# Hippogriff/parsenet-codebase

Hardware: AMD Instinct MI355X
Metric: shapes/sec fwd+bwd on 10k-pt clouds (higher is better)
Workload: dtype f32; 1 GPU; cfg5: ParSeNet e2e (seg + mean-shift 10 it. + per-segment spline/primitive fit + Chamfer/residual), 10k pts, batch 4 per GPU, fwd+bwd+allreduce+Adam; batch_per_gpu=4, points=10000, k=80, parallelism=dp1, global_batch=4

## Files before the change

include/parsenet_hip.h:

```cpp
#ifndef PARSENET_HIP_H
#define PARSENET_HIP_H

#include <stddef.h>
#include <stdint.h>

#ifdef __cplusplus
extern "C" {
#endif

#define PN_OK 0
#define PN_ERR_ARG (-1)
#define PN_ERR_HIP (-2)
#define PN_ERR_WORKSPACE (-3)
#define PN_ERR_UNSUPPORTED (-4)

const char* pn_last_error(void);
int pn_abi_version(void);

void pn_prof_enable(int on);
void pn_prof_reset(void);
int pn_prof_count(void);
int pn_prof_get(int i, char* name, int name_len, double* total_ms, long long* calls);

size_t pn_knn_workspace(int B, int C, int N, int k);
// ... 68 lines not shown
                                int64_t* nearest, void* workspace, size_t workspace_bytes, void* stream);
size_t pn_gemm_x3_weight_image_bytes(int M, int K);
size_t pn_gemm_x3_points_image_bytes(int B, int C, int N);
int pn_gemm_x3_weight_image_f32(const float* w, int M, int K, int transposed, void* img, void* stream);
int pn_gemm_x3_f32(const void* img_a, const float* x, const float* bias, int B, int M, int K, int N, float* out,
                   void* workspace, size_t workspace_bytes, void* stream);
int pn_gemm_x3_cat_f32(const void* img_a, const float* const* xs, const int* cs, int nsrc, const float* bias, int B,
                       int M, int N, float* out, void* workspace, size_t workspace_bytes, void* stream);
size_t pn_gemm_x3_wgrad_workspace(int B, int M, int K, int N);
int pn_gemm_x3_wgrad_f32(const float* gy, const float* x, int B, int M, int K, int N, float* gw, float* gb,
                         void* workspace, size_t workspace_bytes, void* stream);
size_t pn_meanshift_rows_bwd_workspace(int B, int N);
int pn_meanshift_rows_bwd_f32(const float* gy, const float* y, const float* q, const float* rsum, const float* unorm,
                              const float* x, const float* bsq, int B, int N, int D, int R, float* gq, float* gx,
                              void* workspace, size_t workspace_bytes, void* stream);
int pn_meanshift_rows_scatter_add_f32(const float* g, const int64_t* rows, int B, int N, int D, int R, float* gx,
                                      void* stream);
size_t pn_meanshift_x3_plan_bytes(int B, int N);
size_t pn_meanshift_x3_plan_core_bytes(int B, int N);
int pn_kmeans_assign_f32(const float* x, const float* cen, int B, int N, int D, int K, int* lab, void* stream);
int pn_kmeans_centres_f32(const float* x, const int* lab, const float* old, int B, int N, int D, int K,
                          float* cen, void* stream);
int pn_cell_order_i32(const int* rank, const int* home, const int* fine, int B, int N, int P, int F,
                      long long* perm, void* stream);
int pn_meanshift_x3_tileinfo_f32(const float* z, int B, int N, int D, float* cen, float* rho, float* cnt,
                                 void* stream);
int pn_meanshift_x3_plan_f32(const float* cenQ, const float* rhoQ, const float* cenX, const float* rhoX,
                             const float* cntX, const float* bsq, int B, int N, float rel_eps, void* plan,
                             void* stream);
int pn_meanshift_x3_iter_fwd_plan_f32(const float* q, const void* img_x, const float* bsq, int B, int N,
// ... 208 lines not shown
```

parsenet_codebase_amd/_lib.py:

```python
import ctypes
import os

import torch

_HERE = os.path.dirname(os.path.abspath(__file__))
LIB_PATH = os.path.join(_HERE, "libparsenet_hip.so")

c_void_p = ctypes.c_void_p
c_int = ctypes.c_int
c_float = ctypes.c_float
c_size_t = ctypes.c_size_t
c_double = ctypes.c_double

ABI_VERSION = 22

SIGNATURES = {
    "pn_last_error": (ctypes.c_char_p, []),
    "pn_abi_version": (c_int, []),
    "pn_prof_enable": (None, [c_int]),
    "pn_prof_reset": (None, []),
    "pn_prof_count": (c_int, []),
    "pn_prof_get": (c_int, [c_int, ctypes.c_char_p, c_int, ctypes.POINTER(c_double),
                            ctypes.POINTER(ctypes.c_longlong)]),
    "pn_knn_workspace": (c_size_t, [c_int, c_int, c_int, c_int]),
    "pn_knn_f32": (c_int, [c_void_p, c_int, c_int, c_int, c_int, c_void_p, c_void_p, c_size_t, c_void_p]),
    "pn_knn_pn_f32": (c_int, [c_void_p, c_int, c_int, c_int, c_void_p, c_void_p, c_size_t, c_void_p]),
    "pn_knn_graph_i32": (c_int, [c_void_p, c_int, c_int, c_int, c_int, c_int, c_void_p, c_void_p, c_size_t, c_void_p]),
    "pn_knn3_ragged": (c_int, [c_void_p, c_void_p, c_int, c_int, c_int, c_int, c_void_p, c_void_p, c_void_p]),
    "pn_transpose_f32": (c_int, [c_void_p, c_void_p, c_int, c_int, c_int, c_void_p]),
# ... 55 lines not shown
                               c_void_p]),
    "pn_standardize_select_f32": (c_int, [c_void_p, c_int, c_int, c_int, c_void_p, c_void_p]),
    "pn_standardize_scale_f32": (c_int, [c_void_p, c_void_p, c_void_p, c_int, c_int, c_float, c_void_p, c_void_p,
                                         c_void_p]),
    "pn_gather_flat_f32": (c_int, [c_void_p, c_void_p, c_void_p, c_int, c_void_p, c_void_p]),
    "pn_adam_flat_f32": (c_int, [c_void_p, c_void_p, c_void_p, c_void_p, ctypes.c_longlong, ctypes.c_float,
                                 ctypes.c_float, ctypes.c_float, ctypes.c_float, c_int, c_void_p]),
    "pn_gemm_x3_cat_f32": (c_int, [c_void_p, c_void_p, c_void_p, c_int, c_void_p, c_int, c_int, c_int, c_void_p, c_void_p,
                                   c_size_t, c_void_p]),
    "pn_gemm_x3_wgrad_workspace": (c_size_t, [c_int, c_int, c_int, c_int]),
    "pn_gemm_x3_wgrad_f32": (c_int, [c_void_p, c_void_p, c_int, c_int, c_int, c_int, c_void_p, c_void_p, c_void_p,
                                     c_size_t, c_void_p]),
    "pn_meanshift_rows_bwd_workspace": (c_size_t, [c_int, c_int]),
    "pn_meanshift_rows_bwd_f32": (c_int, [c_void_p] * 7 + [c_int, c_int, c_int, c_int, c_void_p, c_void_p, c_void_p,
                                          c_size_t, c_void_p]),
    "pn_meanshift_rows_scatter_add_f32": (c_int, [c_void_p, c_void_p, c_int, c_int, c_int, c_int, c_void_p, c_void_p]),
    "pn_meanshift_x3_plan_bytes": (c_size_t, [c_int, c_int]),
    "pn_meanshift_x3_plan_core_bytes": (c_size_t, [c_int, c_int]),
    "pn_gn_max_finish_f32": (c_int, [c_void_p] * 8 + [c_int, c_int, c_int] + [c_void_p] * 5),
    "pn_gn_max_bwd_prep_f32": (c_int, [c_void_p] * 3 + [c_int, c_int] + [c_void_p] * 3),
    "pn_cell_order_i32": (c_int, [c_void_p, c_void_p, c_void_p, c_int, c_int, c_int, c_int, c_void_p, c_void_p]),
    "pn_kmeans_assign_f32": (c_int, [c_void_p, c_void_p, c_int, c_int, c_int, c_int, c_void_p, c_void_p]),
    "pn_kmeans_centres_f32": (c_int, [c_void_p, c_void_p, c_void_p, c_int, c_int, c_int, c_int, c_void_p, c_void_p]),
    "pn_meanshift_chain_order_f32": (c_int, [c_void_p, c_int, c_int, c_void_p, c_void_p]),
    "pn_meanshift_x3_tileinfo_f32": (c_int, [c_void_p, c_int, c_int, c_int, c_void_p, c_void_p, c_void_p, c_void_p]),
    "pn_meanshift_x3_plan_f32": (c_int, [c_void_p] * 6 + [c_int, c_int, c_float, c_void_p, c_void_p]),
    "pn_meanshift_x3_iter_fwd_plan_f32": (c_int, [c_void_p] * 3 + [c_int, c_int, c_int] + [c_void_p] * 5 +
                                          [c_void_p, c_void_p]),
    "pn_meanshift_x3_iter_fwd_info_f32": (c_int, [c_void_p] * 3 + [c_int, c_int, c_int] + [c_void_p] * 5 +
                                          [c_void_p] * 5),
# ... 295 lines not shown
```

parsenet_codebase_amd/csrc/error.hip:

```cpp
#include "common.h"
#include <stdarg.h>

static thread_local char g_err[512] = "";

void pn_set_error(const char* fmt, ...) {
  va_list ap;
  va_start(ap, fmt);
  vsnprintf(g_err, sizeof(g_err), fmt, ap);
  va_end(ap);
}

extern "C" const char* pn_last_error(void) { return g_err; }

extern "C" int pn_abi_version(void) { return 22; }
```

parsenet_codebase_amd/csrc/meanshift_rows.hip:

```cpp
#include "common.h"
#include <cstdlib>

#define MR_DMAX 128
#define MR_R 64
#define MR_CB 64
#define MR_LDOF(D) ((D) + 4)
#define MR_LG 68
#define MR_LOG2E 1.4426950408889634f
#define MR_LIM2 (75.0f * MR_LOG2E)

__device__ static inline float4 mr_ld4(const float* p) { return *reinterpret_cast<const float4*>(p); }
template <int NV>
__device__ static inline void mr_ldn(const float* p, float* v) {
  if constexpr (NV == 8) {
    const float4 a = mr_ld4(p), b = mr_ld4(p + 4);
    v[0] = a.x; v[1] = a.y; v[2] = a.z; v[3] = a.w;
    v[4] = b.x; v[5] = b.y; v[6] = b.z; v[7] = b.w;
  } else if constexpr (NV == 4) {
    const float4 a = mr_ld4(p);
    v[0] = a.x; v[1] = a.y; v[2] = a.z; v[3] = a.w;
  } else {
    const float2 a = *reinterpret_cast<const float2*>(p);
    v[0] = a.x; v[1] = a.y;
  }
}

template <int MR_D, int MR_LD>
__global__ __launch_bounds__(256) void pn_ms_rows_prep_kernel(const float* __restrict__ gy, const float* __restrict__ y,
                                                              const float* __restrict__ rsum, const float* __restrict__ unorm,
                                                              const float* __restrict__ bsq, int R, float* __restrict__ gu,
                                                              float* __restrict__ scal) {
  const int b = blockIdx.y;
  const int wave = threadIdx.x >> 6, lane = threadIdx.x & 63;
  const int r = blockIdx.x * 4 + wave;
  if (r >= MR_R) return;
  float u0 = 0.f, u1 = 0.f, c = 0.f, al = 0.f, ri = 0.f;
  if (r < R) {
    const size_t base = ((size_t)b * R + r) * MR_D;
    const bool lo = MR_D >= 64 || lane < MR_D;
    float y0 = 0.f, y1 = 0.f, g0 = 0.f, g1 = 0.f;
    if (lo) y0 = y[base + lane];
    if constexpr (MR_D == 128) y1 = y[base + lane + 64];
    if (lo) g0 = gy[base + lane];
    if constexpr (MR_D == 128) g1 = gy[base + lane + 64];
    const float nn = unorm[(size_t)b * R + r], rr = rsum[(size_t)b * R + r];
    const float yg = pn_wave_sum(y0 * g0 + y1 * g1);
    u0 = (g0 - y0 * yg) / nn;
    u1 = (g1 - y1 * yg) / nn;
    c = pn_wave_sum(u0 * (y0 * nn) + u1 * (y1 * nn));
    al = 1.0f / (rr * bsq[b]);
    ri = 1.0f / rr;
  }
  float* g = gu + ((size_t)b * MR_R + r) * MR_D;
  if (lane < MR_D) g[lane] = u0;
  if constexpr (MR_D == 128) g[lane + 64] = u1;
  if (lane == 0) {
    float* sp = scal + ((size_t)b * MR_R + r) * 4;
    sp[0] = c;
    sp[1] = al;
    sp[2] = ri;
    sp[3] = 0.f;
  }
}

template <int MR_D, int MR_LD>
__global__ __launch_bounds__(256) void pn_ms_rows_bwd_kernel(
    const float* __restrict__ gu, const float* __restrict__ scal, const float* __restrict__ q,
    const float* __restrict__ x, const float* __restrict__ bsq, int N, int R, int nblk, float* __restrict__ gx,
    float* __restrict__ gq_part) {
  extern __shared__ __attribute__((aligned(16))) float lds[];
  float* Xs = lds;
  float* Qs = Xs + MR_CB * MR_LD;
  float* Us = Qs + MR_R * MR_LD;
  float* GS = Us + MR_R * MR_LD;
  float* KR = GS + MR_R * MR_LG;
  float* GT = KR + MR_R * MR_LG;
  float* sc = GT + MR_CB * MR_LG;
  float* sa = sc + MR_R;
  float* sr = sa + MR_R;
  const int b = blockIdx.y, blk = blockIdx.x, tid = threadIdx.x;
  constexpr int MR_L4 = MR_D == 128 ? 5 : MR_D == 64 ? 4 : 3;

  const int j0 = blk * MR_CB;
  const float bs = bsq[b];
  const float hl = (0.5f / bs) * MR_LOG2E;
  const float* __restrict__ xb = x + (size_t)b * N * MR_D;

  for (int it = tid; it < MR_CB * (MR_D / 4); it += 256) {
    const int r = it >> MR_L4, c4 = it & (MR_D / 4 - 1);
    float4 v = make_float4(0.f, 0.f, 0.f, 0.f);
    if (j0 + r < N) v = mr_ld4(xb + (size_t)(j0 + r) * MR_D + 4 * c4);
    *reinterpret_cast<float4*>(Xs + r * MR_LD + 4 * c4) = v;
    float4 w = make_float4(0.f, 0.f, 0.f, 0.f);
    if (r < R) w = mr_ld4(q + ((size_t)b * R + r) * MR_D + 4 * c4);
    *reinterpret_cast<float4*>(Qs + r * MR_LD + 4 * c4) = w;
  }
  for (int it = tid; it < MR_R * (MR_D / 4); it += 256) {
    const int r = it >> MR_L4, c4 = it & (MR_D / 4 - 1);
    *reinterpret_cast<float4*>(Us + r * MR_LD + 4 * c4) = mr_ld4(gu + ((size_t)b * MR_R + r) * MR_D + 4 * c4);
  }
  if (tid < MR_R) {
    const float4 sv = mr_ld4(scal + ((size_t)b * MR_R + tid) * 4);
    sc[tid] = sv.x;
    sa[tid] = sv.y;
    sr[tid] = sv.z;
  }
  __syncthreads();

  {
    const int ti = tid >> 4, tj = tid & 15;
    float s[4][4], t[4][4];
#pragma unroll
    for (int a = 0; a < 4; ++a)
#pragma unroll
      for (int e = 0; e < 4; ++e) {
        s[a][e] = 0.f;
        t[a][e] = 0.f;
      }
    for (int k = 0; k < MR_D; k += 4) {
      float4 qv[4], uv[4], xv[4];
#pragma unroll
      for (int a = 0; a < 4; ++a) {
        qv[a] = mr_ld4(Qs + (ti + 16 * a) * MR_LD + k);
        uv[a] = mr_ld4(Us + (ti + 16 * a) * MR_LD + k);
        xv[a] = mr_ld4(Xs + (tj + 16 * a) * MR_LD + k);
      }
#pragma unroll
      for (int a = 0; a < 4; ++a)
#pragma unroll
        for (int e = 0; e < 4; ++e) {
          s[a][e] = __builtin_fmaf(qv[a].x, xv[e].x, s[a][e]);
          s[a][e] = __builtin_fmaf(qv[a].y, xv[e].y, s[a][e]);
          s[a][e] = __builtin_fmaf(qv[a].z, xv[e].z, s[a][e]);
          s[a][e] = __builtin_fmaf(qv[a].w, xv[e].w, s[a][e]);
          t[a][e] = __builtin_fmaf(uv[a].x, xv[e].x, t[a][e]);
          t[a][e] = __builtin_fmaf(uv[a].y, xv[e].y, t[a][e]);
          t[a][e] = __builtin_fmaf(uv[a].z, xv[e].z, t[a][e]);
          t[a][e] = __builtin_fmaf(uv[a].w, xv[e].w, t[a][e]);
        }
    }
#pragma unroll
    for (int a = 0; a < 4; ++a) {
      const int i = ti + 16 * a;
      const float ci = sc[i], ai = sa[i], ri = sr[i];
#pragma unroll
      for (int e = 0; e < 4; ++e) {
        const int j = tj + 16 * e;
        const float dist = __builtin_fmaf(-2.0f, s[a][e], 2.0f);
        const float a2 = -dist * hl;
        const float a2c = __builtin_amdgcn_fmed3f(a2, -MR_LIM2, MR_LIM2);
        float kv = __builtin_amdgcn_exp2f(a2c);
        if (j0 + j >= N) kv = 0.f;
        const float g = a2c == a2 ? kv * ((t[a][e] - ci) * ai) : 0.f;
        GS[i * MR_LG + j] = g;
        GT[j * MR_LG + i] = g;
        KR[i * MR_LG + j] = kv * ri;
      }
    }
  }
  __syncthreads();

  constexpr int NF4 = MR_D / 4;
  constexpr int RPT = MR_CB * NF4 / 256;
  const int f4 = tid & (NF4 - 1), grp = tid >> MR_L4;
  {
    float4 acc[RPT];
#pragma unroll
    for (int e = 0; e < RPT; ++e) acc[e] = make_float4(0.f, 0.f, 0.f, 0.f);
    for (int i = 0; i < MR_R; ++i) {
      const float4 qv = mr_ld4(Qs + i * MR_LD + 4 * f4);
      const float4 uv = mr_ld4(Us + i * MR_LD + 4 * f4);
      float gv[RPT], kv[RPT];
      mr_ldn<RPT>(GS + i * MR_LG + RPT * grp, gv);
      mr_ldn<RPT>(KR + i * MR_LG + RPT * grp, kv);
#pragma unroll
      for (int e = 0; e < RPT; ++e) {
        acc[e].x = __builtin_fmaf(gv[e], qv.x, acc[e].x);
        acc[e].y = __builtin_fmaf(gv[e], qv.y, acc[e].y);
        acc[e].z = __builtin_fmaf(gv[e], qv.z, acc[e].z);
        acc[e].w = __builtin_fmaf(gv[e], qv.w, acc[e].w);
        acc[e].x = __builtin_fmaf(kv[e], uv.x, acc[e].x);
        acc[e].y = __builtin_fmaf(kv[e], uv.y, acc[e].y);
        acc[e].z = __builtin_fmaf(kv[e], uv.z, acc[e].z);
        acc[e].w = __builtin_fmaf(kv[e], uv.w, acc[e].w);
// ... 1 lines not shown
    }
#pragma unroll
    for (int e = 0; e < RPT; ++e) {
      const int j = j0 + RPT * grp + e;
      if (j < N) {
        float4* o = reinterpret_cast<float4*>(gx + ((size_t)b * N + j) * MR_D + 4 * f4);
        float4 v = *o;
        v.x += acc[e].x;
        v.y += acc[e].y;
        v.z += acc[e].z;
        v.w += acc[e].w;
        *o = v;
      }
    }
  }
  {
    float4 acc[RPT];
#pragma unroll
    for (int e = 0; e < RPT; ++e) acc[e] = make_float4(0.f, 0.f, 0.f, 0.f);
    for (int j = 0; j < MR_CB; ++j) {
      const float4 xv = mr_ld4(Xs + j * MR_LD + 4 * f4);
      float gv[RPT];
      mr_ldn<RPT>(GT + j * MR_LG + RPT * grp, gv);
#pragma unroll
      for (int e = 0; e < RPT; ++e) {
        acc[e].x = __builtin_fmaf(gv[e], xv.x, acc[e].x);
        acc[e].y = __builtin_fmaf(gv[e], xv.y, acc[e].y);
        acc[e].z = __builtin_fmaf(gv[e], xv.z, acc[e].z);
        acc[e].w = __builtin_fmaf(gv[e], xv.w, acc[e].w);
      }
    }
    float* pb = gq_part + ((size_t)b * nblk + blk) * MR_R * MR_D;
#pragma unroll
    for (int e = 0; e < RPT; ++e) *reinterpret_cast<float4*>(pb + (RPT * grp + e) * MR_D + 4 * f4) = acc[e];
  }
}

template <int MR_D, int MR_LD>
__global__ __launch_bounds__(256) void pn_ms_rows_reduce_kernel(const float* __restrict__ gq_part, int R, int nblk,
                                                                float* __restrict__ gq) {
  const int b = blockIdx.y;
  const int e = blockIdx.x * 256 + threadIdx.x;
  if (e >= R * (MR_D / 4)) return;
  const float* p = gq_part + (size_t)b * nblk * MR_R * MR_D + 4 * e;
  float4 s = make_float4(0.f, 0.f, 0.f, 0.f);
  int k = 0;
  for (; k + 8 <= nblk; k += 8) {
    float4 v[8];
#pragma unroll
    for (int u = 0; u < 8; ++u) v[u] = mr_ld4(p + (size_t)(k + u) * MR_R * MR_D);
#pragma unroll
    for (int u = 0; u < 8; ++u) {
      s.x += v[u].x;
      s.y += v[u].y;
      s.z += v[u].z;
      s.w += v[u].w;
    }
  }
  for (; k < nblk; ++k) {
    const float4 v = mr_ld4(p + (size_t)k * MR_R * MR_D);
    s.x += v.x;
    s.y += v.y;
    s.z += v.z;
    s.w += v.w;
  }
  *reinterpret_cast<float4*>(gq + (size_t)b * R * MR_D + 4 * e) = s;
}

template <int MR_D, int MR_LD>
__global__ __launch_bounds__(256) void pn_ms_rows_scatter_kernel(const float* __restrict__ g, const int64_t* __restrict__ rows,
                                                                 int N, int R, float* __restrict__ gx) {
  const int b = blockIdx.x, tid = threadIdx.x;
  const int f4 = tid & 31, sub = tid >> 5;
  for (int r0 = 0; r0 < R; r0 += 8) {
    for (int turn = 0; turn < 8; ++turn) {
      const int r = r0 + turn;
      if (sub == turn && r < R && f4 < MR_D / 4) {
        const int64_t row = rows[(size_t)b * R + r];
        if (row >= 0 && row < N) {
          float4* o = reinterpret_cast<float4*>(gx + ((size_t)b * N + row) * MR_D + 4 * f4);
          const float4 v = mr_ld4(g + ((size_t)b * R + r) * MR_D + 4 * f4);
// ... 6 lines not shown
        }
      }
      __syncthreads();
    }
  }
}

static size_t mr_part_bytes(int B, int N) {
  return pn_align_up((size_t)B * pn_cdiv(N, MR_CB) * MR_R * MR_DMAX * sizeof(float), 256);
}
static size_t mr_gu_bytes(int B) { return pn_align_up((size_t)B * MR_R * MR_DMAX * sizeof(float), 256); }
extern "C" size_t pn_meanshift_rows_bwd_workspace(int B, int N) {
  return mr_part_bytes(B, N) + mr_gu_bytes(B) + pn_align_up((size_t)B * MR_R * 4 * sizeof(float), 256);
}

template <int MR_D>
static int mr_rows_bwd(const float* gy, const float* y, const float* q, const float* rsum, const float* unorm,
                       const float* x, const float* bsq, int B, int N, int R, float* gq, float* gx, void* workspace,
                       hipStream_t stream) {
  constexpr int MR_LD = MR_LDOF(MR_D);
  const int nblk = pn_cdiv(N, MR_CB);
  const size_t lds_valu = (size_t)(3 * MR_R * MR_LD + 3 * MR_R * MR_LG + 3 * MR_R) * sizeof(float);
  static unsigned attr_devs = 0;
  if (pn_first_on_device(&attr_devs)) {
    PN_CHECK_HIP(hipFuncSetAttribute(reinterpret_cast<const void*>(pn_ms_rows_bwd_kernel<MR_D, MR_LD>),
                                     hipFuncAttributeMaxDynamicSharedMemorySize, (int)lds_valu));
  }
  float* part = static_cast<float*>(workspace);
  float* gu = reinterpret_cast<float*>(static_cast<char*>(workspace) + mr_part_bytes(B, N));
  float* scal = reinterpret_cast<float*>(static_cast<char*>(workspace) + mr_part_bytes(B, N) + mr_gu_bytes(B));
  {
    PN_PROF("meanshift_rows_bwd", stream);
    hipLaunchKernelGGL((pn_ms_rows_prep_kernel<MR_D, MR_LD>), dim3(MR_R / 4, B), dim3(256), 0, stream, gy, y, rsum, unorm,
                       bsq, R, gu, scal);
    hipLaunchKernelGGL((pn_ms_rows_bwd_kernel<MR_D, MR_LD>), dim3(nblk, B), dim3(256), lds_valu, stream, (const float*)gu,
                       (const float*)scal, q, x, bsq, N, R, nblk, gx, part);
  }
  PN_CHECK_LAUNCH();
  hipLaunchKernelGGL((pn_ms_rows_reduce_kernel<MR_D, MR_LD>), dim3(pn_cdiv(R * (MR_D / 4), 256), B), dim3(256), 0, stream,
                     (const float*)part, R, nblk, gq);
  PN_CHECK_LAUNCH();
  return PN_OK;
}

extern "C" int pn_meanshift_rows_bwd_f32(const float* gy, const float* y, const float* q, const float* rsum,
                                         const float* unorm, const float* x, const float* bsq, int B, int N, int D,
                                         int R, float* gq, float* gx, void* workspace, size_t workspace_bytes,
                                         hipStream_t stream) {
  PN_CHECK_ARG(D == 32 || D == 64 || D == 128, "pn_meanshift_rows_bwd_f32: D must be one of {32, 64, 128}, got %d", D);
  PN_CHECK_ARG(R >= 1 && R <= MR_R, "pn_meanshift_rows_bwd_f32: 1 <= R <= %d, got %d", MR_R, R);
  PN_CHECK_ARG(B >= 1 && N >= 1, "pn_meanshift_rows_bwd_f32: empty input");
  if (workspace_bytes < pn_meanshift_rows_bwd_workspace(B, N)) {
    pn_set_error("pn_meanshift_rows_bwd_f32: workspace too small");
    return PN_ERR_WORKSPACE;
  }
  if (D == 32) return mr_rows_bwd<32>(gy, y, q, rsum, unorm, x, bsq, B, N, R, gq, gx, workspace, stream);
  if (D == 64) return mr_rows_bwd<64>(gy, y, q, rsum, unorm, x, bsq, B, N, R, gq, gx, workspace, stream);
  return mr_rows_bwd<128>(gy, y, q, rsum, unorm, x, bsq, B, N, R, gq, gx, workspace, stream);
}

extern "C" int pn_meanshift_rows_scatter_add_f32(const float* g, const int64_t* rows, int B, int N, int D, int R,
                                                 float* gx, hipStream_t stream) {
  PN_CHECK_ARG(D == 32 || D == 64 || D == 128, "pn_meanshift_rows_scatter_add_f32: D must be one of {32, 64, 128}, got %d",
               D);
  PN_CHECK_ARG(B >= 1 && R >= 1, "pn_meanshift_rows_scatter_add_f32: empty input");
  if (D == 32)
    hipLaunchKernelGGL((pn_ms_rows_scatter_kernel<32, MR_LDOF(32)>), dim3(B), dim3(256), 0, stream, g, rows, N, R, gx);
  else if (D == 64)
    hipLaunchKernelGGL((pn_ms_rows_scatter_kernel<64, MR_LDOF(64)>), dim3(B), dim3(256), 0, stream, g, rows, N, R, gx);
  else
    hipLaunchKernelGGL((pn_ms_rows_scatter_kernel<128, MR_LDOF(128)>), dim3(B), dim3(256), 0, stream, g, rows, N, R, gx);
  PN_CHECK_LAUNCH();
  return PN_OK;
// ... 2 lines not shown
```

parsenet_codebase_amd/kernels.py:

```python
import torch

from . import _lib
from ._lib import check, current_stream, ptr, require_cuda


def _f32c(t, name):
    if t.dtype != torch.float32:
        raise TypeError("%s must be float32, got %s" % (name, t.dtype))
    return t.contiguous()


def chamfer_nn(a, b, side_a=True, side_b=True):
    require_cuda(a, b)
    a = _f32c(a, "a")
    b = _f32c(b, "b")
    if a.dim() != 3 or b.dim() != 3 or a.shape[2] != 3 or b.shape[2] != 3 or a.shape[0] != b.shape[0]:
        raise ValueError("chamfer_nn expects (B,Na,3) and (B,Nb,3), got %s and %s"
                         % (tuple(a.shape), tuple(b.shape)))
    B, Na, _ = a.shape
    Nb = b.shape[1]
    if Na == 0 or Nb == 0 or B == 0:
        raise ValueError("chamfer_nn: empty cloud")
    lib = _lib.load()
    dev = a.device
# ... 719 lines not shown
        raise ValueError("meanshift_rows_bwd: rsum, unorm (B,R), gx (B,N,D)")
    if gx.dtype != torch.float32 or not gx.is_contiguous():
        raise TypeError("meanshift_rows_bwd: gx must be contiguous fp32")
    lib = _lib.load()
    wsz = lib.pn_meanshift_rows_bwd_workspace(B, N)
    if ws is None or ws.numel() < wsz:
        ws = torch.empty(wsz, dtype=torch.uint8, device=x.device)
    gq = torch.empty_like(q)
    with _lib.on_device(x.device):
        rc = lib.pn_meanshift_rows_bwd_f32(ptr(gy), ptr(y), ptr(q), ptr(rsum), ptr(unorm), ptr(x), ptr(bsq), B, N, D, R,
                                           ptr(gq), ptr(gx), ptr(ws), ws.numel(), current_stream(x.device))
    check(rc, "pn_meanshift_rows_bwd_f32")
    return gq


def meanshift_rows_workspace(B, N, device):
    return torch.empty(_lib.load().pn_meanshift_rows_bwd_workspace(B, N), dtype=torch.uint8, device=device)


def meanshift_rows_scatter_add(gx, rows, g):
    require_cuda(gx, rows, g)
    g = _f32c(g, "g")
    rows = _i64c(rows, "rows")
    B, N, D = gx.shape
    R = rows.shape[1]
    if tuple(g.shape) != (B, R, D) or gx.dtype != torch.float32 or not gx.is_contiguous():
        raise ValueError("meanshift_rows_scatter_add: g (B,R,D), gx contiguous fp32 (B,N,D)")
    with _lib.on_device(gx.device):
        rc = _lib.load().pn_meanshift_rows_scatter_add_f32(ptr(g), ptr(rows), B, N, D, R, ptr(gx),
                                                           current_stream(gx.device))
# ... 437 lines not shown
```

parsenet_codebase_amd/mean_shift.py:

```python
import os

import numpy as np
import torch

from . import kernels as K
from ._lib import h2d, require_cuda


ARITH = os.environ.get("PARSENET_MS_ARITH", "bf16x3")
_env_sparse = os.environ.get("PARSENET_MS_SPARSE", "auto")
SPARSE = True if _env_sparse == "1" else False if _env_sparse == "0" else "auto"
AUTO_DENSE_ABOVE = 0.93
AUTO_DENSE_STEPS = 48
AUTO_SAMPLES = 4
_AUTO = {}
CALLS = {"planned": 0, "dense": 0}
AUTO_STAT = None
PLAN_REL_EPS = float(os.environ.get("PARSENET_MS_REL_EPS", "1e-6"))
PLAN_REL_EPS_DENSE_BWD = float(os.environ.get("PARSENET_MS_REL_EPS_BWD", str(min(PLAN_REL_EPS, 1e-9))))
SPARSE_MIN_N = 2048
SPARSE_MAX_N = 32768
LAST_PLAN_STATS = None
WANT_NEAREST = False
LAST_NEAREST = None
# ... 342 lines not shown
        R = rows.shape[1]
        Qc = torch.gather(state.iterates, 2, rows.view(1, B, R, 1).expand(T + 1, B, R, D))
        rc = torch.gather(state.rsums, 2, rows.view(1, B, R).expand(T, B, R))
        nc = torch.gather(state.norms, 2, rows.view(1, B, R).expand(T, B, R))
        ctx.T = T
        ctx.has_inv = state.inv is not None
        ctx.save_for_backward(Qc, rc, nc, rows, state.x, state.bsq, *([state.inv] if state.inv is not None else []))
        return Qc[T].clone()

    @staticmethod
    def backward(ctx, g):
        Qc, rc, nc, rows, x, bsq = ctx.saved_tensors[:6]
        B, N, D = x.shape
        gX = torch.zeros_like(x)
        g = g.contiguous()
        ws = K.meanshift_rows_workspace(B, N, x.device)
        for t in reversed(range(ctx.T)):
            g = K.meanshift_rows_bwd(g, Qc[t + 1], Qc[t], rc[t], nc[t], x, bsq, gX, ws)
        K.meanshift_rows_scatter_add(gX, rows, g)
        if ctx.has_inv:
            inv = ctx.saved_tensors[6]
            gX = torch.gather(gX, 1, inv.unsqueeze(2).expand(-1, -1, D))
        return gX, None, None


def centre_rows(X, state, ids):
    if ids.shape[1] > 64:
        raise ValueError("centre_rows: at most 64 rows per batch item, got %d" % ids.shape[1])
    return _CentreRows.apply(X, state, ids)


def _first_argmax(vals, dim):
    m = vals.max(dim, keepdim=True)[0]
# ... 142 lines not shown
```

Baseline: 176.6 shapes/s.

## Fuse mean-shift row backward over all iterations and skip zero-gradient rows

Replaces the per-iteration Python loop of mean-shift row backward calls with one library entry that launches all T iterations back-to-back. The reduce kernel now also prepares the next iteration's gradient and scalars, which removes the separate prep kernel. A first kernel compacts rows whose incoming gradient is nonzero so the main kernel only computes products for live rows, with tile sizes picked at runtime. This cuts launch and host overhead and skips dead-row work, at the cost of more template variants and index-compaction logic.

New measurement: 182.7 shapes/s (median of 6 runs). +3.4%, better.

```diff
diff --git a/include/parsenet_hip.h b/include/parsenet_hip.h
--- a/include/parsenet_hip.h
+++ b/include/parsenet_hip.h
@@ -106,6 +106,9 @@
 int pn_meanshift_rows_bwd_f32(const float* gy, const float* y, const float* q, const float* rsum, const float* unorm,
                               const float* x, const float* bsq, int B, int N, int D, int R, float* gq, float* gx,
                               void* workspace, size_t workspace_bytes, void* stream);
+int pn_meanshift_rows_bwd_all_f32(const float* gy, const float* Qc, const float* rsums, const float* norms,
+                                  const float* x, const float* bsq, int B, int N, int D, int R, int T, float* gq,
+                                  float* gx, void* workspace, size_t workspace_bytes, void* stream);
 int pn_meanshift_rows_scatter_add_f32(const float* g, const int64_t* rows, int B, int N, int D, int R, float* gx,
                                       void* stream);
 size_t pn_meanshift_x3_plan_bytes(int B, int N);
diff --git a/parsenet_codebase_amd/_lib.py b/parsenet_codebase_amd/_lib.py
--- a/parsenet_codebase_amd/_lib.py
+++ b/parsenet_codebase_amd/_lib.py
@@ -12,7 +12,7 @@
 c_size_t = ctypes.c_size_t
 c_double = ctypes.c_double
 
-ABI_VERSION = 22
+ABI_VERSION = 23
 
 SIGNATURES = {
     "pn_last_error": (ctypes.c_char_p, []),
@@ -98,6 +98,8 @@
     "pn_meanshift_rows_bwd_workspace": (c_size_t, [c_int, c_int]),
     "pn_meanshift_rows_bwd_f32": (c_int, [c_void_p] * 7 + [c_int, c_int, c_int, c_int, c_void_p, c_void_p, c_void_p,
                                           c_size_t, c_void_p]),
+    "pn_meanshift_rows_bwd_all_f32": (c_int, [c_void_p] * 6 + [c_int, c_int, c_int, c_int, c_int, c_void_p, c_void_p,
+                                              c_void_p, c_size_t, c_void_p]),
     "pn_meanshift_rows_scatter_add_f32": (c_int, [c_void_p, c_void_p, c_int, c_int, c_int, c_int, c_void_p, c_void_p]),
     "pn_meanshift_x3_plan_bytes": (c_size_t, [c_int, c_int]),
     "pn_meanshift_x3_plan_core_bytes": (c_size_t, [c_int, c_int]),
diff --git a/parsenet_codebase_amd/csrc/error.hip b/parsenet_codebase_amd/csrc/error.hip
--- a/parsenet_codebase_amd/csrc/error.hip
+++ b/parsenet_codebase_amd/csrc/error.hip
@@ -12,4 +12,4 @@
 
 extern "C" const char* pn_last_error(void) { return g_err; }
 
-extern "C" int pn_abi_version(void) { return 22; }
+extern "C" int pn_abi_version(void) { return 23; }
diff --git a/parsenet_codebase_amd/csrc/meanshift_rows.hip b/parsenet_codebase_amd/csrc/meanshift_rows.hip
--- a/parsenet_codebase_amd/csrc/meanshift_rows.hip
+++ b/parsenet_codebase_amd/csrc/meanshift_rows.hip
@@ -19,52 +19,173 @@
   } else if constexpr (NV == 4) {
     const float4 a = mr_ld4(p);
     v[0] = a.x; v[1] = a.y; v[2] = a.z; v[3] = a.w;
-  } else {
+  } else if constexpr (NV == 2) {
     const float2 a = *reinterpret_cast<const float2*>(p);
     v[0] = a.x; v[1] = a.y;
-  }
-}
-
-template <int MR_D, int MR_LD>
-__global__ __launch_bounds__(256) void pn_ms_rows_prep_kernel(const float* __restrict__ gy, const float* __restrict__ y,
-                                                              const float* __restrict__ rsum, const float* __restrict__ unorm,
-                                                              const float* __restrict__ bsq, int R, float* __restrict__ gu,
-                                                              float* __restrict__ scal) {
-  const int b = blockIdx.y;
-  const int wave = threadIdx.x >> 6, lane = threadIdx.x & 63;
-  const int r = blockIdx.x * 4 + wave;
-  if (r >= MR_R) return;
-  float u0 = 0.f, u1 = 0.f, c = 0.f, al = 0.f, ri = 0.f;
-  if (r < R) {
-    const size_t base = ((size_t)b * R + r) * MR_D;
-    const bool lo = MR_D >= 64 || lane < MR_D;
-    float y0 = 0.f, y1 = 0.f, g0 = 0.f, g1 = 0.f;
-    if (lo) y0 = y[base + lane];
-    if constexpr (MR_D == 128) y1 = y[base + lane + 64];
-    if (lo) g0 = gy[base + lane];
-    if constexpr (MR_D == 128) g1 = gy[base + lane + 64];
-    const float nn = unorm[(size_t)b * R + r], rr = rsum[(size_t)b * R + r];
-    const float yg = pn_wave_sum(y0 * g0 + y1 * g1);
-    u0 = (g0 - y0 * yg) / nn;
-    u1 = (g1 - y1 * yg) / nn;
-    c = pn_wave_sum(u0 * (y0 * nn) + u1 * (y1 * nn));
-    al = 1.0f / (rr * bsq[b]);
-    ri = 1.0f / rr;
-  }
-  float* g = gu + ((size_t)b * MR_R + r) * MR_D;
+  } else {
+    v[0] = p[0];
+  }
+}
+
+template <int MR_D>
+__device__ static inline void mr_prep_row(float g0, float g1, const float* __restrict__ yrow, float nn, float rr, float bs,
+                                          int lane, float* __restrict__ g, float* __restrict__ sp) {
+  const bool lo = MR_D >= 64 || lane < MR_D;
+  float y0 = 0.f, y1 = 0.f;
+  if (lo) y0 = yrow[lane];
+  if constexpr (MR_D == 128) y1 = yrow[lane + 64];
+  const float yg = pn_wave_sum(y0 * g0 + y1 * g1);
+  const float u0 = (g0 - y0 * yg) / nn;
+  const float u1 = (g1 - y1 * yg) / nn;
+  const float c = pn_wave_sum(u0 * (y0 * nn) + u1 * (y1 * nn));
   if (lane < MR_D) g[lane] = u0;
   if constexpr (MR_D == 128) g[lane + 64] = u1;
   if (lane == 0) {
-    float* sp = scal + ((size_t)b * MR_R + r) * 4;
     sp[0] = c;
-    sp[1] = al;
-    sp[2] = ri;
-    sp[3] = 0.f;
-  }
-}
-
-template <int MR_D, int MR_LD>
-__global__ __launch_bounds__(256) void pn_ms_rows_bwd_kernel(
+    sp[1] = 1.0f / (rr * bs);
+    sp[2] = 1.0f / rr;
+  }
+}
+
+template <int MR_D>
+__device__ static inline void mr_prep_none(int lane, float* __restrict__ g, float* __restrict__ sp) {
+  if (lane < MR_D) g[lane] = 0.f;
+  if constexpr (MR_D == 128) g[lane + 64] = 0.f;
+  if (lane == 0) {
+    sp[0] = 0.f;
+    sp[1] = 0.f;
+    sp[2] = 0.f;
+    reinterpret_cast<int*>(sp)[3] = -1;
+  }
+}
+
+template <int MR_D>
+__global__ __launch_bounds__(1024) void pn_ms_rows_first_kernel(const float* __restrict__ gy, const float* __restrict__ y,
+                                                                const float* __restrict__ rsum,
+                                                                const float* __restrict__ unorm,
+                                                                const float* __restrict__ bsq, int R, int all_live,
+                                                                float* __restrict__ gu, float* __restrict__ scal) {
+  __shared__ int flag[MR_R];
+  const int b = blockIdx.x;
+  const int wave = threadIdx.x >> 6, lane = threadIdx.x & 63;
+  const bool lo = MR_D >= 64 || lane < MR_D;
+  for (int r = wave; r < MR_R; r += 16) {
+    bool nz = false;
+    if (r < R) {
+      const size_t base = ((size_t)b * R + r) * MR_D;
+      float g0 = 0.f, g1 = 0.f;
+      if (lo) g0 = gy[base + lane];
+      if constexpr (MR_D == 128) g1 = gy[base + lane + 64];
+      nz = all_live || __ballot(g0 != 0.f || g1 != 0.f) != 0ull;
+    }
+    if (lane == 0) flag[r] = nz ? 1 : 0;
+  }
+  __syncthreads();
+  const bool mine = flag[lane] != 0;
+  const unsigned long long mask = __ballot(mine);
+  const int L = __popcll(mask);
+  const int rank = pn_mbcnt(mask);
+  for (int p = wave; p < MR_R; p += 16) {
+    float* g = gu + ((size_t)b * MR_R + p) * MR_D;
+    float* sp = scal + ((size_t)b * MR_R + p) * 4;
+    if (p >= L) {
+      mr_prep_none<MR_D>(lane, g, sp);
+      continue;
+    }
+    const int r = __ffsll(__ballot(mine && rank == p)) - 1;
+    const size_t base = ((size_t)b * R + r) * MR_D;
+    float g0 = 0.f, g1 = 0.f;
+    if (lo) g0 = gy[base + lane];
+    if constexpr (MR_D == 128) g1 = gy[base + lane + 64];
+    mr_prep_row<MR_D>(g0, g1, y + base, unorm[(size_t)b * R + r], rsum[(size_t)b * R + r], bsq[b], lane, g, sp);
+    if (lane == 0) reinterpret_cast<int*>(sp)[3] = r;
+  }
+}
+
+template <int MR_D, int MR_LD, int NA>
+__device__ static inline void mr_block_products(const float* Xs, const float* Qs, const float* Us, float* GS, float* KR,
+                                                float* GT, const float* sc, const float* sa, const float* sr, int tid,
+                                                int j0, int N, float hl) {
+  const int ti = tid >> 4, tj = tid & 15;
+  float s[NA][4], t[NA][4];
+#pragma unroll
+  for (int a = 0; a < NA; ++a)
+#pragma unroll
+    for (int e = 0; e < 4; ++e) {
+      s[a][e] = 0.f;
+      t[a][e] = 0.f;
+    }
+#pragma unroll 2
+  for (int k = 0; k < MR_D; k += 4) {
+    float4 qv[NA], uv[NA], xv[4];
+#pragma unroll
+    for (int a = 0; a < NA; ++a) {
+      qv[a] = mr_ld4(Qs + (ti + 16 * a) * MR_LD + k);
+      uv[a] = mr_ld4(Us + (ti + 16 * a) * MR_LD + k);
+    }
+#pragma unroll
+    for (int e = 0; e < 4; ++e) xv[e] = mr_ld4(Xs + (tj + 16 * e) * MR_LD + k);
+#pragma unroll
+    for (int a = 0; a < NA; ++a)
+#pragma unroll
+      for (int e = 0; e < 4; ++e) {
+        s[a][e] = __builtin_fmaf(qv[a].x, xv[e].x, s[a][e]);
+        s[a][e] = __builtin_fmaf(qv[a].y, xv[e].y, s[a][e]);
+        s[a][e] = __builtin_fmaf(qv[a].z, xv[e].z, s[a][e]);
+        s[a][e] = __builtin_fmaf(qv[a].w, xv[e].w, s[a][e]);
+        t[a][e] = __builtin_fmaf(uv[a].x, xv[e].x, t[a][e]);
+        t[a][e] = __builtin_fmaf(uv[a].y, xv[e].y, t[a][e]);
+        t[a][e] = __builtin_fmaf(uv[a].z, xv[e].z, t[a][e]);
+        t[a][e] = __builtin_fmaf(uv[a].w, xv[e].w, t[a][e]);
+      }
+  }
+#pragma unroll
+  for (int a = 0; a < NA; ++a) {
+    const int i = ti + 16 * a;
+    const float ci = sc[i], ai = sa[i], ri = sr[i];
+#pragma unroll
+    for (int e = 0; e < 4; ++e) {
+      const int j = tj + 16 * e;
+      const float dist = __builtin_fmaf(-2.0f, s[a][e], 2.0f);
+      const float a2 = -dist * hl;
+      const float a2c = __builtin_amdgcn_fmed3f(a2, -MR_LIM2, MR_LIM2);
+      float kv = __builtin_amdgcn_exp2f(a2c);
+      if (j0 + j >= N) kv = 0.f;
+      const float g = a2c == a2 ? kv * ((t[a][e] - ci) * ai) : 0.f;
+      GS[i * MR_LG + j] = g;
+      GT[j * MR_LG + i] = g;
+      KR[i * MR_LG + j] = kv * ri;
+    }
+  }
+}
+
+template <int MR_D, int NR>
+__device__ static inline void mr_gq_partial(const float* Xs, const float* GT, float* __restrict__ pb, int tid, int L) {
+  constexpr int MR_LD = MR_LDOF(MR_D), NF4 = MR_D / 4;
+  constexpr int MR_L4 = MR_D == 128 ? 5 : MR_D == 64 ? 4 : 3;
+  const int f4 = tid & (NF4 - 1), grp = tid >> MR_L4;
+  if (NR * grp >= L) return;
+  float4 acc[NR];
+#pragma unroll
+  for (int e = 0; e < NR; ++e) acc[e] = make_float4(0.f, 0.f, 0.f, 0.f);
+  for (int j = 0; j < MR_CB; ++j) {
+    const float4 xv = mr_ld4(Xs + j * MR_LD + 4 * f4);
+    float gv[NR];
+    mr_ldn<NR>(GT + j * MR_LG + NR * grp, gv);
+#pragma unroll
+    for (int e = 0; e < NR; ++e) {
+      acc[e].x = __builtin_fmaf(gv[e], xv.x, acc[e].x);
+      acc[e].y = __builtin_fmaf(gv[e], xv.y, acc[e].y);
+      acc[e].z = __builtin_fmaf(gv[e], xv.z, acc[e].z);
+      acc[e].w = __builtin_fmaf(gv[e], xv.w, acc[e].w);
+    }
+  }
+#pragma unroll
+  for (int e = 0; e < NR; ++e) *reinterpret_cast<float4*>(pb + (NR * grp + e) * MR_D + 4 * f4) = acc[e];
+}
+
+template <int MR_D, int MR_LD, bool LIVE>
+__global__ __launch_bounds__(256) __attribute__((amdgpu_waves_per_eu(MR_D == 32 ? 2 : 1))) void pn_ms_rows_bwd_kernel(
     const float* __restrict__ gu, const float* __restrict__ scal, const float* __restrict__ q,
     const float* __restrict__ x, const float* __restrict__ bsq, int N, int R, int nblk, float* __restrict__ gx,
     float* __restrict__ gq_part) {
@@ -81,6 +202,14 @@
   const int b = blockIdx.y, blk = blockIdx.x, tid = threadIdx.x;
   constexpr int MR_L4 = MR_D == 128 ? 5 : MR_D == 64 ? 4 : 3;
 
+  int L = MR_R;
+  if constexpr (LIVE) {
+    const int row = reinterpret_cast<const int*>(scal)[((size_t)b * MR_R + (tid & 63)) * 4 + 3];
+    L = __popcll(__ballot(row >= 0));
+    if (L == 0) return;
+  }
+  const int LP = LIVE ? (L + 15) & ~15 : MR_R;
+
   const int j0 = blk * MR_CB;
   const float bs = bsq[b];
   const float hl = (0.5f / bs) * MR_LOG2E;
@@ -91,15 +220,23 @@
     float4 v = make_float4(0.f, 0.f, 0.f, 0.f);
     if (j0 + r < N) v = mr_ld4(xb + (size_t)(j0 + r) * MR_D + 4 * c4);
     *reinterpret_cast<float4*>(Xs + r * MR_LD + 4 * c4) = v;
-    float4 w = make_float4(0.f, 0.f, 0.f, 0.f);
-    if (r < R) w = mr_ld4(q + ((size_t)b * R + r) * MR_D + 4 * c4);
-    *reinterpret_cast<float4*>(Qs + r * MR_LD + 4 * c4) = w;
-  }
-  for (int it = tid; it < MR_R * (MR_D / 4); it += 256) {
+    if constexpr (!LIVE) {
+      float4 w = make_float4(0.f, 0.f, 0.f, 0.f);
+      if (r < R) w = mr_ld4(q + ((size_t)b * R + r) * MR_D + 4 * c4);
+      *reinterpret_cast<float4*>(Qs + r * MR_LD + 4 * c4) = w;
+    }
+  }
+  for (int it = tid; it < LP * (MR_D / 4); it += 256) {
     const int r = it >> MR_L4, c4 = it & (MR_D / 4 - 1);
     *reinterpret_cast<float4*>(Us + r * MR_LD + 4 * c4) = mr_ld4(gu + ((size_t)b * MR_R + r) * MR_D + 4 * c4);
-  }
-  if (tid < MR_R) {
+    if constexpr (LIVE) {
+      const int row = reinterpret_cast<const int*>(scal)[((size_t)b * MR_R + r) * 4 + 3];
+      float4 w = make_float4(0.f, 0.f, 0.f, 0.f);
+      if (row >= 0 && row < R) w = mr_ld4(q + ((size_t)b * R + row) * MR_D + 4 * c4);
+      *reinterpret_cast<float4*>(Qs + r * MR_LD + 4 * c4) = w;
+    }
+  }
+  if (tid < LP) {
     const float4 sv = mr_ld4(scal + ((size_t)b * MR_R + tid) * 4);
     sc[tid] = sv.x;
     sa[tid] = sv.y;
@@ -107,56 +244,13 @@
   }
   __syncthreads();
 
-  {
-    const int ti = tid >> 4, tj = tid & 15;
-    float s[4][4], t[4][4];
-#pragma unroll
-    for (int a = 0; a < 4; ++a)
-#pragma unroll
-      for (int e = 0; e < 4; ++e) {
-        s[a][e] = 0.f;
-        t[a][e] = 0.f;
-      }
-    for (int k = 0; k < MR_D; k += 4) {
-      float4 qv[4], uv[4], xv[4];
-#pragma unroll
-      for (int a = 0; a < 4; ++a) {
-        qv[a] = mr_ld4(Qs + (ti + 16 * a) * MR_LD + k);
-        uv[a] = mr_ld4(Us + (ti + 16 * a) * MR_LD + k);
-        xv[a] = mr_ld4(Xs + (tj + 16 * a) * MR_LD + k);
-      }
-#pragma unroll
-      for (int a = 0; a < 4; ++a)
-#pragma unroll
-        for (int e = 0; e < 4; ++e) {
-          s[a][e] = __builtin_fmaf(qv[a].x, xv[e].x, s[a][e]);
-          s[a][e] = __builtin_fmaf(qv[a].y, xv[e].y, s[a][e]);
-          s[a][e] = __builtin_fmaf(qv[a].z, xv[e].z, s[a][e]);
-          s[a][e] = __builtin_fmaf(qv[a].w, xv[e].w, s[a][e]);
-          t[a][e] = __builtin_fmaf(uv[a].x, xv[e].x, t[a][e]);
-          t[a][e] = __builtin_fmaf(uv[a].y, xv[e].y, t[a][e]);
-          t[a][e] = __builtin_fmaf(uv[a].z, xv[e].z, t[a][e]);
-          t[a][e] = __builtin_fmaf(uv[a].w, xv[e].w, t[a][e]);
-        }
-    }
-#pragma unroll
-    for (int a = 0; a < 4; ++a) {
-      const int i = ti + 16 * a;
-      const float ci = sc[i], ai = sa[i], ri = sr[i];
-#pragma unroll
-      for (int e = 0; e < 4; ++e) {
-        const int j = tj + 16 * e;
-        const float dist = __builtin_fmaf(-2.0f, s[a][e], 2.0f);
-        const float a2 = -dist * hl;
-        const float a2c = __builtin_amdgcn_fmed3f(a2, -MR_LIM2, MR_LIM2);
-        float kv = __builtin_amdgcn_exp2f(a2c);
-        if (j0 + j >= N) kv = 0.f;
-        const float g = a2c == a2 ? kv * ((t[a][e] - ci) * ai) : 0.f;
-        GS[i * MR_LG + j] = g;
-        GT[j * MR_LG + i] = g;
-        KR[i * MR_LG + j] = kv * ri;
-      }
-    }
+  if constexpr (LIVE) {
+    if (LP == 16) mr_block_products<MR_D, MR_LD, 1>(Xs, Qs, Us, GS, KR, GT, sc, sa, sr, tid, j0, N, hl);
+    else if (LP == 32) mr_block_products<MR_D, MR_LD, 2>(Xs, Qs, Us, GS, KR, GT, sc, sa, sr, tid, j0, N, hl);
+    else if (LP == 48) mr_block_products<MR_D, MR_LD, 3>(Xs, Qs, Us, GS, KR, GT, sc, sa, sr, tid, j0, N, hl);
+    else mr_block_products<MR_D, MR_LD, 4>(Xs, Qs, Us, GS, KR, GT, sc, sa, sr, tid, j0, N, hl);
+  } else {
+    mr_block_products<MR_D, MR_LD, 4>(Xs, Qs, Us, GS, KR, GT, sc, sa, sr, tid, j0, N, hl);
   }
   __syncthreads();
 
@@ -167,7 +261,7 @@
     float4 acc[RPT];
 #pragma unroll
     for (int e = 0; e < RPT; ++e) acc[e] = make_float4(0.f, 0.f, 0.f, 0.f);
-    for (int i = 0; i < MR_R; ++i) {
+    for (int i = 0; i < L; ++i) {
       const float4 qv = mr_ld4(Qs + i * MR_LD + 4 * f4);
       const float4 uv = mr_ld4(Us + i * MR_LD + 4 * f4);
       float gv[RPT], kv[RPT];
@@ -199,57 +293,73 @@
       }
     }
   }
-  {
-    float4 acc[RPT];
-#pragma unroll
-    for (int e = 0; e < RPT; ++e) acc[e] = make_float4(0.f, 0.f, 0.f, 0.f);
-    for (int j = 0; j < MR_CB; ++j) {
-      const float4 xv = mr_ld4(Xs + j * MR_LD + 4 * f4);
-      float gv[RPT];
-      mr_ldn<RPT>(GT + j * MR_LG + RPT * grp, gv);
-#pragma unroll
-      for (int e = 0; e < RPT; ++e) {
-        acc[e].x = __builtin_fmaf(gv[e], xv.x, acc[e].x);
-        acc[e].y = __builtin_fmaf(gv[e], xv.y, acc[e].y);
-        acc[e].z = __builtin_fmaf(gv[e], xv.z, acc[e].z);
-        acc[e].w = __builtin_fmaf(gv[e], xv.w, acc[e].w);
+  float* pb = gq_part + ((size_t)b * nblk + blk) * MR_R * MR_D;
+  if constexpr (LIVE) {
+    constexpr int NG = 256 / NF4;
+    if (L <= NG) mr_gq_partial<MR_D, 1>(Xs, GT, pb, tid, L);
+    else if (L <= 2 * NG || RPT == 2) mr_gq_partial<MR_D, 2>(Xs, GT, pb, tid, L);
+    else if (L <= 4 * NG || RPT == 4) mr_gq_partial<MR_D, (RPT >= 4 ? 4 : RPT)>(Xs, GT, pb, tid, L);
+    else mr_gq_partial<MR_D, RPT>(Xs, GT, pb, tid, L);
+  } else {
+    mr_gq_partial<MR_D, RPT>(Xs, GT, pb, tid, L);
+  }
+}
+
+template <int MR_D>
+__global__ __launch_bounds__(256) void pn_ms_rows_reduce_kernel(const float* __restrict__ gq_part, int R, int nblk,
+                                                                const float* __restrict__ y, const float* __restrict__ rsum,
+                                                                const float* __restrict__ unorm,
+                                                                const float* __restrict__ bsq, float* __restrict__ gq,
+                                                                float* __restrict__ gu, float* __restrict__ scal) {
+  constexpr int NF4 = MR_D / 4;
+  const int b = blockIdx.y;
+  const int wave = threadIdx.x >> 6, lane = threadIdx.x & 63;
+  const int p = blockIdx.x * 4 + wave;
+  if (p >= MR_R) return;
+  const int lrow = reinterpret_cast<const int*>(scal)[((size_t)b * MR_R + lane) * 4 + 3];
+  if (gq != nullptr && p < R && __ballot(lrow == p) == 0ull && lane < NF4)
+    *reinterpret_cast<float4*>(gq + ((size_t)b * R + p) * MR_D + 4 * lane) = make_float4(0.f, 0.f, 0.f, 0.f);
+  const int row = __shfl(lrow, p, 64);
+  if (row < 0 || row >= R) return;
+  float4 s = make_float4(0.f, 0.f, 0.f, 0.f);
+  if (lane < NF4) {
+    const float* pp = gq_part + (size_t)b * nblk * MR_R * MR_D + (size_t)p * MR_D + 4 * lane;
+    int k = 0;
+    for (; k + 8 <= nblk; k += 8) {
+      float4 v[8];
+#pragma unroll
+      for (int u = 0; u < 8; ++u) v[u] = mr_ld4(pp + (size_t)(k + u) * MR_R * MR_D);
+#pragma unroll
+      for (int u = 0; u < 8; ++u) {
+        s.x += v[u].x;
+        s.y += v[u].y;
+        s.z += v[u].z;
+        s.w += v[u].w;
       }
     }
-    float* pb = gq_part + ((size_t)b * nblk + blk) * MR_R * MR_D;
-#pragma unroll
-    for (int e = 0; e < RPT; ++e) *reinterpret_cast<float4*>(pb + (RPT * grp + e) * MR_D + 4 * f4) = acc[e];
-  }
-}
-
-template <int MR_D, int MR_LD>
-__global__ __launch_bounds__(256) void pn_ms_rows_reduce_kernel(const float* __restrict__ gq_part, int R, int nblk,
-                                                                float* __restrict__ gq) {
-  const int b = blockIdx.y;
-  const int e = blockIdx.x * 256 + threadIdx.x;
-  if (e >= R * (MR_D / 4)) return;
-  const float* p = gq_part + (size_t)b * nblk * MR_R * MR_D + 4 * e;
-  float4 s = make_float4(0.f, 0.f, 0.f, 0.f);
-  int k = 0;
-  for (; k + 8 <= nblk; k += 8) {
-    float4 v[8];
-#pragma unroll
-    for (int u = 0; u < 8; ++u) v[u] = mr_ld4(p + (size_t)(k + u) * MR_R * MR_D);
-#pragma unroll
-    for (int u = 0; u < 8; ++u) {
-      s.x += v[u].x;
-      s.y += v[u].y;
-      s.z += v[u].z;
-      s.w += v[u].w;
-    }
-  }
-  for (; k < nblk; ++k) {
-    const float4 v = mr_ld4(p + (size_t)k * MR_R * MR_D);
-    s.x += v.x;
-    s.y += v.y;
-    s.z += v.z;
-    s.w += v.w;
-  }
-  *reinterpret_cast<float4*>(gq + (size_t)b * R * MR_D + 4 * e) = s;
+    for (; k < nblk; ++k) {
+      const float4 v = mr_ld4(pp + (size_t)k * MR_R * MR_D);
+      s.x += v.x;
+      s.y += v.y;
+      s.z += v.z;
+      s.w += v.w;
+    }
+    if (gq != nullptr) *reinterpret_cast<float4*>(gq + ((size_t)b * R + row) * MR_D + 4 * lane) = s;
+  }
+  if (y == nullptr) return;
+  const int c = lane & 3;
+  const int s0 = lane >> 2;
+  const float a0 = __shfl(s.x, s0, 64), a1 = __shfl(s.y, s0, 64), a2 = __shfl(s.z, s0, 64), a3 = __shfl(s.w, s0, 64);
+  const float g0 = c == 0 ? a0 : c == 1 ? a1 : c == 2 ? a2 : a3;
+  float g1 = 0.f;
+  if constexpr (MR_D == 128) {
+    const int s1 = 16 + (lane >> 2);
+    const float b0 = __shfl(s.x, s1, 64), b1 = __shfl(s.y, s1, 64), b2 = __shfl(s.z, s1, 64), b3 = __shfl(s.w, s1, 64);
+    g1 = c == 0 ? b0 : c == 1 ? b1 : c == 2 ? b2 : b3;
+  }
+  const size_t base = ((size_t)b * R + row) * MR_D;
+  mr_prep_row<MR_D>(g0, g1, y + base, unorm[(size_t)b * R + row], rsum[(size_t)b * R + row], bsq[b], lane,
+                    gu + ((size_t)b * MR_R + p) * MR_D, scal + ((size_t)b * MR_R + p) * 4);
 }
 
 template <int MR_D, int MR_LD>
@@ -286,49 +396,83 @@
   return mr_part_bytes(B, N) + mr_gu_bytes(B) + pn_align_up((size_t)B * MR_R * 4 * sizeof(float), 256);
 }
 
+static bool mr_live_rows() {
+  const char* e = getenv("PARSENET_MS_ROWS_LIVE");
+  return !(e && e[0] == '0' && e[1] == 0);
+}
+
 template <int MR_D>
-static int mr_rows_bwd(const float* gy, const float* y, const float* q, const float* rsum, const float* unorm,
-                       const float* x, const float* bsq, int B, int N, int R, float* gq, float* gx, void* workspace,
-                       hipStream_t stream) {
+static int mr_rows_bwd_all(const float* gy, const float* ylast, const float* Qc, const float* rsums, const float* norms, const float* x,
+                           const float* bsq, int B, int N, int R, int T, float* gq, float* gx, void* workspace,
+                           hipStream_t stream) {
   constexpr int MR_LD = MR_LDOF(MR_D);
   const int nblk = pn_cdiv(N, MR_CB);
   const size_t lds_valu = (size_t)(3 * MR_R * MR_LD + 3 * MR_R * MR_LG + 3 * MR_R) * sizeof(float);
+  const bool live = mr_live_rows();
   static unsigned attr_devs = 0;
   if (pn_first_on_device(&attr_devs)) {
-    PN_CHECK_HIP(hipFuncSetAttribute(reinterpret_cast<const void*>(pn_ms_rows_bwd_kernel<MR_D, MR_LD>),
+    PN_CHECK_HIP(hipFuncSetAttribute(reinterpret_cast<const void*>(pn_ms_rows_bwd_kernel<MR_D, MR_LD, true>),
+                                     hipFuncAttributeMaxDynamicSharedMemorySize, (int)lds_valu));
+    PN_CHECK_HIP(hipFuncSetAttribute(reinterpret_cast<const void*>(pn_ms_rows_bwd_kernel<MR_D, MR_LD, false>),
                                      hipFuncAttributeMaxDynamicSharedMemorySize, (int)lds_valu));
   }
   float* part = static_cast<float*>(workspace);
   float* gu = reinterpret_cast<float*>(static_cast<char*>(workspace) + mr_part_bytes(B, N));
   float* scal = reinterpret_cast<float*>(static_cast<char*>(workspace) + mr_part_bytes(B, N) + mr_gu_bytes(B));
-  {
+  const size_t rows = (size_t)B * R, it = rows * MR_D;
+  for (int t = T - 1; t >= 0; --t) {
     PN_PROF("meanshift_rows_bwd", stream);
-    hipLaunchKernelGGL((pn_ms_rows_prep_kernel<MR_D, MR_LD>), dim3(MR_R / 4, B), dim3(256), 0, stream, gy, y, rsum, unorm,
-                       bsq, R, gu, scal);
-    hipLaunchKernelGGL((pn_ms_rows_bwd_kernel<MR_D, MR_LD>), dim3(nblk, B), dim3(256), lds_valu, stream, (const float*)gu,
-                       (const float*)scal, q, x, bsq, N, R, nblk, gx, part);
-  }
-  PN_CHECK_LAUNCH();
-  hipLaunchKernelGGL((pn_ms_rows_reduce_kernel<MR_D, MR_LD>), dim3(pn_cdiv(R * (MR_D / 4), 256), B), dim3(256), 0, stream,
-                     (const float*)part, R, nblk, gq);
-  PN_CHECK_LAUNCH();
+    if (t == T - 1)
+      hipLaunchKernelGGL((pn_ms_rows_first_kernel<MR_D>), dim3(B), dim3(1024), 0, stream, gy, ylast,
+                         rsums + (size_t)t * rows, norms + (size_t)t * rows, bsq, R, live ? 0 : 1, gu, scal);
+    if (live)
+      hipLaunchKernelGGL((pn_ms_rows_bwd_kernel<MR_D, MR_LD, true>), dim3(nblk, B), dim3(256), lds_valu, stream,
+                         (const float*)gu, (const float*)scal, Qc + (size_t)t * it, x, bsq, N, R, nblk, gx, part);
+    else
+      hipLaunchKernelGGL((pn_ms_rows_bwd_kernel<MR_D, MR_LD, false>), dim3(nblk, B), dim3(256), lds_valu, stream,
+                         (const float*)gu, (const float*)scal, Qc + (size_t)t * it, x, bsq, N, R, nblk, gx, part);
+    if (t > 0)
+      hipLaunchKernelGGL((pn_ms_rows_reduce_kernel<MR_D>), dim3(MR_R / 4, B), dim3(256), 0, stream, (const float*)part,
+                         R, nblk, Qc + (size_t)t * it, rsums + (size_t)(t - 1) * rows, norms + (size_t)(t - 1) * rows, bsq,
+                         (float*)nullptr, gu, scal);
+    else
+      hipLaunchKernelGGL((pn_ms_rows_reduce_kernel<MR_D>), dim3(MR_R / 4, B), dim3(256), 0, stream, (const float*)part,
+                         R, nblk, (const float*)nullptr, (const float*)nullptr, (const float*)nullptr, bsq, gq, gu, scal);
+    PN_CHECK_LAUNCH();
+  }
   return PN_OK;
+}
+
+static int mr_check(const char* who, int B, int N, int D, int R, size_t workspace_bytes) {
+  PN_CHECK_ARG(D == 32 || D == 64 || D == 128, "%s: D must be one of {32, 64, 128}, got %d", who, D);
+  PN_CHECK_ARG(R >= 1 && R <= MR_R, "%s: 1 <= R <= %d, got %d", who, MR_R, R);
+  PN_CHECK_ARG(B >= 1 && N >= 1, "%s: empty input", who);
+  if (workspace_bytes < pn_meanshift_rows_bwd_workspace(B, N)) {
+    pn_set_error("%s: workspace too small", who);
+    return PN_ERR_WORKSPACE;
+  }
+  return PN_OK;
+}
+
+extern "C" int pn_meanshift_rows_bwd_all_f32(const float* gy, const float* Qc, const float* rsums, const float* norms,
+                                             const float* x, const float* bsq, int B, int N, int D, int R, int T,
+                                             float* gq, float* gx, void* workspace, size_t workspace_bytes,
+                                             hipStream_t stream) {
+  if (const int rc = mr_check("pn_meanshift_rows_bwd_all_f32", B, N, D, R, workspace_bytes)) return rc;
+  PN_CHECK_ARG(T >= 1, "pn_meanshift_rows_bwd_all_f32: T >= 1, got %d", T);
+  if (D == 32) return mr_rows_bwd_all<32>(gy, Qc + (size_t)T * B * R * D, Qc, rsums, norms, x, bsq, B, N, R, T, gq, gx, workspace, stream);
+  if (D == 64) return mr_rows_bwd_all<64>(gy, Qc + (size_t)T * B * R * D, Qc, rsums, norms, x, bsq, B, N, R, T, gq, gx, workspace, stream);
+  return mr_rows_bwd_all<128>(gy, Qc + (size_t)T * B * R * D, Qc, rsums, norms, x, bsq, B, N, R, T, gq, gx, workspace, stream);
 }
 
 extern "C" int pn_meanshift_rows_bwd_f32(const float* gy, const float* y, const float* q, const float* rsum,
                                          const float* unorm, const float* x, const float* bsq, int B, int N, int D,
                                          int R, float* gq, float* gx, void* workspace, size_t workspace_bytes,
                                          hipStream_t stream) {
-  PN_CHECK_ARG(D == 32 || D == 64 || D == 128, "pn_meanshift_rows_bwd_f32: D must be one of {32, 64, 128}, got %d", D);
-  PN_CHECK_ARG(R >= 1 && R <= MR_R, "pn_meanshift_rows_bwd_f32: 1 <= R <= %d, got %d", MR_R, R);
-  PN_CHECK_ARG(B >= 1 && N >= 1, "pn_meanshift_rows_bwd_f32: empty input");
-  if (workspace_bytes < pn_meanshift_rows_bwd_workspace(B, N)) {
-    pn_set_error("pn_meanshift_rows_bwd_f32: workspace too small");
-    return PN_ERR_WORKSPACE;
-  }
-  if (D == 32) return mr_rows_bwd<32>(gy, y, q, rsum, unorm, x, bsq, B, N, R, gq, gx, workspace, stream);
-  if (D == 64) return mr_rows_bwd<64>(gy, y, q, rsum, unorm, x, bsq, B, N, R, gq, gx, workspace, stream);
-  return mr_rows_bwd<128>(gy, y, q, rsum, unorm, x, bsq, B, N, R, gq, gx, workspace, stream);
+  if (const int rc = mr_check("pn_meanshift_rows_bwd_f32", B, N, D, R, workspace_bytes)) return rc;
+  if (D == 32) return mr_rows_bwd_all<32>(gy, y, q, rsum, unorm, x, bsq, B, N, R, 1, gq, gx, workspace, stream);
+  if (D == 64) return mr_rows_bwd_all<64>(gy, y, q, rsum, unorm, x, bsq, B, N, R, 1, gq, gx, workspace, stream);
+  return mr_rows_bwd_all<128>(gy, y, q, rsum, unorm, x, bsq, B, N, R, 1, gq, gx, workspace, stream);
 }
 
 extern "C" int pn_meanshift_rows_scatter_add_f32(const float* g, const int64_t* rows, int B, int N, int D, int R,
diff --git a/parsenet_codebase_amd/kernels.py b/parsenet_codebase_amd/kernels.py
--- a/parsenet_codebase_amd/kernels.py
+++ b/parsenet_codebase_amd/kernels.py
@@ -757,6 +757,31 @@
     return gq
 
 
+def meanshift_rows_bwd_all(gy, Qc, rsums, norms, x, bsq, gx, ws=None):
+    require_cuda(gy, Qc, rsums, norms, x, bsq, gx)
+    gy, Qc, x = _f32c(gy, "gy"), _f32c(Qc, "Qc"), _f32c(x, "x")
+    rsums, norms, bsq = _f32c(rsums, "rsums"), _f32c(norms, "norms"), _f32c(bsq, "bsq")
+    B, N, D = x.shape
+    R = gy.shape[1]
+    T = rsums.shape[0]
+    if tuple(gy.shape) != (B, R, D) or tuple(Qc.shape) != (T + 1, B, R, D):
+        raise ValueError("meanshift_rows_bwd_all: gy (B,R,D), Qc (T+1,B,R,D)")
+    if tuple(rsums.shape) != (T, B, R) or tuple(norms.shape) != (T, B, R) or tuple(gx.shape) != (B, N, D):
+        raise ValueError("meanshift_rows_bwd_all: rsums, norms (T,B,R), gx (B,N,D)")
+    if gx.dtype != torch.float32 or not gx.is_contiguous():
+        raise TypeError("meanshift_rows_bwd_all: gx must be contiguous fp32")
+    lib = _lib.load()
+    wsz = lib.pn_meanshift_rows_bwd_workspace(B, N)
+    if ws is None or ws.numel() < wsz:
+        ws = torch.empty(wsz, dtype=torch.uint8, device=x.device)
+    gq = torch.empty_like(gy)
+    with _lib.on_device(x.device):
+        rc = lib.pn_meanshift_rows_bwd_all_f32(ptr(gy), ptr(Qc), ptr(rsums), ptr(norms), ptr(x), ptr(bsq), B, N, D, R, T,
+                                               ptr(gq), ptr(gx), ptr(ws), ws.numel(), current_stream(x.device))
+    check(rc, "pn_meanshift_rows_bwd_all_f32")
+    return gq
+
+
 def meanshift_rows_workspace(B, N, device):
     return torch.empty(_lib.load().pn_meanshift_rows_bwd_workspace(B, N), dtype=torch.uint8, device=device)
 
diff --git a/parsenet_codebase_amd/mean_shift.py b/parsenet_codebase_amd/mean_shift.py
--- a/parsenet_codebase_amd/mean_shift.py
+++ b/parsenet_codebase_amd/mean_shift.py
@@ -380,9 +380,8 @@
         B, N, D = x.shape
         gX = torch.zeros_like(x)
         g = g.contiguous()
-        ws = K.meanshift_rows_workspace(B, N, x.device)
-        for t in reversed(range(ctx.T)):
-            g = K.meanshift_rows_bwd(g, Qc[t + 1], Qc[t], rc[t], nc[t], x, bsq, gX, ws)
+        if ctx.T > 0:
+            g = K.meanshift_rows_bwd_all(g, Qc, rc, nc, x, bsq, gX)
         K.meanshift_rows_scatter_add(gX, rows, g)
         if ctx.has_inv:
             inv = ctx.saved_tensors[6]
```
